# ruc-aimc-lab/GeoFormer

Measured on AMD Instinct MI355X. Metric: image-pairs/sec (640x640), higher is better.
Workload: dtype f16

## Files before the change

### geoformer_amd/_lib.py

```python
import ctypes
import os

_HERE = os.path.dirname(os.path.abspath(__file__))
LIB_PATH = os.environ.get('GF_LIB_PATH') or os.path.join(_HERE, 'libgeoformer_hip.so')

GF_F32, GF_F16, GF_BF16 = 0, 1, 2
GF_IMAGE_U8, GF_IMAGE_F32_NORMALISED, GF_IMAGE_F32_NORMALISED_RCP = 0, 1, 2

c_void_p, c_int, c_float, c_size_t = ctypes.c_void_p, ctypes.c_int, ctypes.c_float, ctypes.c_size_t
c_long, c_uint32 = ctypes.c_long, ctypes.c_uint32

SIGNATURES = {
    'gf_abi_version': (c_int, []),
    'gf_last_error': (ctypes.c_char_p, []),
    'gf_profile_filter': (None, [ctypes.c_char_p]),
    'gf_profile_enable': (None, [c_int]),
    'gf_profile_collect': (c_int, [ctypes.c_char_p, ctypes.POINTER(ctypes.c_double), ctypes.POINTER(c_int),
                                   ctypes.POINTER(ctypes.c_double)]),
    'gf_dual_softmax_workspace_bytes': (c_size_t, [c_int, c_int, c_int]),
    'gf_dual_softmax_match_only_supported': (c_int, [c_int, c_int, c_int, c_int, c_int, c_int]),
    'gf_dual_softmax_conf_at': (c_int, [c_void_p, c_void_p, c_int, c_int, c_int, c_int, c_int, c_float, c_void_p, c_void_p, c_void_p, c_int,
                                        c_void_p, c_void_p, c_size_t, c_void_p]),
    'gf_dual_softmax_match': (c_int, [c_void_p, c_void_p, c_int, c_int, c_int, c_int, c_int, c_void_p, c_void_p,
                                      c_float, c_float, c_int, c_int, c_int, c_float, c_void_p, c_void_p, c_void_p,
# ... 28 lines not shown
    'gf_coarse_loss_backward': (c_int, [c_int, c_int, c_int, c_int, c_void_p, c_void_p, c_float, c_void_p, c_void_p, c_void_p, c_int, c_void_p, c_float,
                                         c_void_p, c_void_p, c_void_p, c_void_p, c_size_t, c_void_p]),
    'gf_pos_encode': (c_int, [c_void_p, c_int, c_long, c_long, c_long, c_long, c_void_p, c_void_p, c_int, c_int, c_int,
                              c_int, c_int, c_void_p]),
    'gf_linear_attention_workspace_bytes': (c_size_t, [c_int, c_int, c_int, c_int]),
    'gf_linear_attention': (c_int, [c_void_p, c_void_p, c_void_p, c_int, c_int, c_int, c_int, c_int, c_int, c_long,
                                    c_long, c_long, c_void_p, c_void_p, c_float, c_void_p, c_void_p, c_size_t,
                                    c_void_p]),
    'gf_encoder_kv_workspace_bytes': (c_size_t, [c_int, c_int]),
    'gf_encoder_kv_state': (c_int, [c_void_p, c_long, c_int, c_int, c_int, c_void_p, c_void_p, c_void_p, c_void_p, c_size_t, c_void_p]),
    'gf_encoder_layer': (c_int, [c_void_p, c_long, c_void_p, c_long, c_void_p, c_int, c_void_p, c_float, c_void_p, c_void_p, c_float,
                                 c_float, c_int, c_void_p, c_int, c_void_p, c_long, c_int, c_int, c_int, c_void_p]),
    'gf_encoder_layer_kv': (c_int, [c_void_p, c_long, c_void_p, c_int, c_void_p, c_float, c_void_p, c_void_p, c_float, c_float, c_int,
                                    c_void_p, c_long, c_int, c_int, c_int, c_void_p, c_int, c_void_p, c_void_p, c_size_t, c_void_p]),
    'gf_fine_layer': (c_int, [c_void_p, c_void_p, c_void_p, c_int, c_int, c_int, c_void_p, c_void_p, c_float, c_float, c_float, c_void_p]),
    'gf_conv3x3_supported': (c_int, [c_int, c_int]),
    'gf_conv3x3s2_supported': (c_int, [c_int, c_int]),
    'gf_lateral_supported': (c_int, [c_int, c_int]),
    'gf_lateral_upsample_add_nhwc': (c_int, [c_void_p, c_void_p, c_void_p, c_void_p, c_int, c_int, c_int, c_int, c_int, c_int, c_int, c_int, c_void_p]),
    'gf_conv3x3_nhwc': (c_int, [c_void_p, c_void_p, c_void_p, c_void_p, c_void_p, c_void_p, c_int, c_int, c_int, c_int, c_int, c_int,
                                c_float, c_int, c_void_p]),
    'gf_linear': (c_int, [c_void_p, c_long, c_int, c_void_p, c_long, c_int, c_void_p, c_void_p, c_void_p, c_int, c_int,
                          c_void_p, c_void_p, c_float, c_void_p, c_long, c_void_p, c_int, c_void_p, c_long, c_int, c_int,
                          c_int, c_void_p]),
    'gf_ransac_workspace_bytes': (c_size_t, [c_int, c_int]),
    'gf_ransac_homography': (c_int, [c_void_p, c_void_p, c_void_p, c_int, c_int, c_float, c_void_p, c_void_p, c_float,
                                     c_int, c_uint32, c_int, c_int, c_void_p, c_void_p, c_void_p, c_void_p, c_void_p, c_void_p,
                                     c_void_p, c_void_p, c_size_t, c_void_p]),
    'gf_ransac_homography_v2': (c_int, [c_void_p, c_void_p, c_void_p, c_int, c_int, c_float, c_void_p, c_void_p, c_float,
                                        c_int, c_uint32, c_int, c_int, c_void_p, c_void_p, c_void_p, c_void_p, c_void_p, c_void_p,
# ... 115 lines not shown
```

### geoformer_amd/csrc/k11_fine_layer.hip

```cpp
#include <math.h>

#include <type_traits>

#include "gf_common.h"

#ifndef K11_TRACE
#define K11_TRACE 0
#endif
#if K11_TRACE
__device__ long long k11_trace[256 * 8 * 4 * 8];
#define K11_T(slot) do { if ((ln & 63) == 0 && blockIdx.x < 256 && git < 4) k11_trace[((blockIdx.x * 8 + wave) * 4 + git) * 8 + (slot)] = (long long)__builtin_amdgcn_s_memtime(); } while (0)
extern "C" int gf_debug_k11_trace(long long* out) {
    return (int)hipMemcpyFromSymbol(out, HIP_SYMBOL(k11_trace), sizeof(long long) * 256 * 8 * 4 * 8);
}
#else
#define K11_T(slot)
#endif

namespace {

constexpr int FC = 128;
#ifndef K11_FW
#define K11_FW 8
#endif
constexpr int FW = K11_FW;
static_assert(FW == 8 || FW == 4, "a weight block is 4 FW fragments: every wave moves four of them");
constexpr int FRAG = 1024, WBLK = 4 * FW * FRAG;
constexpr int NBLK = 320 / (4 * FW);
constexpr int TILE = 8192;
constexpr int X_OFF = 0;
constexpr int W_OFF = FW * TILE;
constexpr int VEC_OFF = W_OFF + 2 * WBLK;
constexpr int LDS_BYTES = VEC_OFF + 4 * FC * 4;

struct FlArgs {
    const void* x;
    const void* src;
    void* out;
    const void* wstream;
    const float* ln;
    float eps1, eps2, attn_eps;
    int Nw, Lw, groups;
};

template <typename T>
__device__ __forceinline__ typename Mma32<T>::Frag fl_pack8(float a0, float a1, float a2, float a3, float a4, float a5, float a6, float a7) {
    typename Mma32<T>::Frag f;
    f[0] = gf_from_float<T>(a0); f[1] = gf_from_float<T>(a1); f[2] = gf_from_float<T>(a2); f[3] = gf_from_float<T>(a3);
    f[4] = gf_from_float<T>(a4); f[5] = gf_from_float<T>(a5); f[6] = gf_from_float<T>(a6); f[7] = gf_from_float<T>(a7);
    return f;
}
template <typename T>
__device__ __forceinline__ typename Mma32<T>::Frag fl_pack_step(const v16f& a, int s) {
    return s == 0 ? fl_pack8<T>(a[0], a[1], a[2], a[3], a[4], a[5], a[6], a[7])
                  : fl_pack8<T>(a[8], a[9], a[10], a[11], a[12], a[13], a[14], a[15]);
}
__device__ __forceinline__ float fl_phi(float x) {
    return fmaxf(x, 0.f) + __builtin_amdgcn_fmed3f(__builtin_amdgcn_exp2f(x * 1.44269504088896341f), 0.f, 1.f);
}
template <typename T>
__device__ __forceinline__ float fl_rnd(float x) { return gf_to_float(gf_from_float<T>(x)); }

__device__ __forceinline__ v16f fl_zero() { return v16f{0.f, 0.f, 0.f, 0.f, 0.f, 0.f, 0.f, 0.f, 0.f, 0.f, 0.f, 0.f, 0.f, 0.f, 0.f, 0.f}; }

struct FlRing {
    GfRsrc ws;
    char* smem;
    int wave, lane;
    int blk;
    int sblk;
    int total;
};
__device__ __forceinline__ void fl_dma_block(const FlRing& r, int g, int sb) {
    char* dst = r.smem + W_OFF + (g & 1) * WBLK + r.wave * 4 * FRAG;
#pragma unroll
    for (int i = 0; i < 4; ++i) gf_lds_dma(r.ws, dst + i * FRAG, r.lane * 16, sb * WBLK + (r.wave * 4 + i) * FRAG);
    __builtin_amdgcn_sched_barrier(0);
}
template <typename Frag>
__device__ __forceinline__ void fl_load_step(const FlRing& r, Frag (&f)[4], int g, int st) {
    const char* p = r.smem + W_OFF + (g & 1) * WBLK + st * 4 * FRAG + r.lane * 16;
#pragma unroll
    for (int i = 0; i < 4; ++i) f[i] = *reinterpret_cast<const Frag*>(p + i * FRAG);
}
template <typename Frag>
__device__ __forceinline__ void fl_fetch_next(FlRing& r, Frag (&nx)[4], int st) {
    if (st == FW - 1) {
        asm volatile("s_waitcnt vmcnt(0) lgkmcnt(0)" ::: "memory");
        __builtin_amdgcn_s_barrier();
        if (r.blk + 2 < r.total) {
            int sb = r.sblk + 2;
            sb = sb >= NBLK ? sb - NBLK : sb;
            fl_dma_block(r, r.blk + 2, sb);
        }
        if (r.blk + 1 < r.total) fl_load_step(r, nx, r.blk + 1, 0);
        ++r.blk;
        r.sblk = r.sblk + 1 == NBLK ? 0 : r.sblk + 1;
    } else {
        fl_load_step(r, nx, r.blk, st + 1);
    }
}

__device__ __forceinline__ void fl_tile_dma(const GfRsrc& wins, int win_byte_offset, int Lw, char* tile, int lane) {
#pragma unroll
    for (int i = 0; i < 8; ++i) {
        const int row = 8 * (i & 3) + (lane >> 3), slot = lane & 7, c = slot ^ ((row >> 1) & 7);
        const int r = row < Lw ? row : Lw - 1;
        gf_lds_dma(wins, tile + i * FRAG, r * (FC * 2) + (i >> 2) * 128 + c * 16, win_byte_offset);
    }
}

template <typename T>
__global__ __launch_bounds__(64 * FW, 2) void fine_layer(FlArgs a) {
    using Mm = Mma32<T>;
    using Frag = typename Mm::Frag;
    extern __shared__ __attribute__((aligned(16))) char smem[];
    const int tid = threadIdx.x, lane = tid & 63, wave = __builtin_amdgcn_readfirstlane(tid >> 6);
    float* vec = reinterpret_cast<float*>(smem + VEC_OFF);
    char* tile = smem + X_OFF + wave * TILE;
#ifdef K11_PRIO
    if (wave >= 4) __builtin_amdgcn_s_setprio(1);
#endif
    const int my_groups = (a.groups - (int)blockIdx.x + (int)gridDim.x - 1) / (int)gridDim.x;
    FlRing ring{gf_rsrc(a.wstream, (unsigned)NBLK * WBLK), smem, wave, lane, 0, 0, my_groups * NBLK};
    const GfRsrc xrs = gf_rsrc(a.x, (unsigned)a.Nw * a.Lw * (FC * 2)), srs = gf_rsrc(a.src, (unsigned)a.Nw * a.Lw * (FC * 2));
    fl_dma_block(ring, 0, 0);
    fl_dma_block(ring, 1, 1);
    for (int i = tid; i < 4 * FC; i += 64 * FW) vec[i] = a.ln[i];
    const bool same_src = a.src == a.x;
    const float inv_s = 1.0f / (float)a.Lw, eps_s = a.attn_eps * inv_s;
    Frag ones;
#pragma unroll
    for (int j = 0; j < 8; ++j) ones[j] = gf_from_float<T>(1.0f);
    Frag fa[4], fb[4];
    bool first = true;

#define FL_STEP_BEGIN(gs)                                               \
    Frag (&cur)[4] = ((gs) & 1) ? fb : fa;                               \
    Frag (&nxt)[4] = ((gs) & 1) ? fa : fb;                               \
    fl_fetch_next(ring, nxt, (gs) & (FW - 1))

    int git = -1;
    (void)git;
    for (int g = blockIdx.x; g < a.groups; g += gridDim.x) {
        ++git;
        int ln = lane;
        asm volatile("" : "+v"(ln));
        const int h2 = ln >> 5, lr = ln & 31;
        v4u pm0, pm1;
#pragma unroll
        for (int p4 = 0; p4 < 4; ++p4) {
            const int ra = 8 * (p4 >> 1) + 4 * h2 + 2 * (p4 & 1);
            pm0[p4] = (ra < a.Lw ? 0xFFFFu : 0u) | (ra + 1 < a.Lw ? 0xFFFF0000u : 0u);
            pm1[p4] = (ra + 16 < a.Lw ? 0xFFFFu : 0u) | (ra + 17 < a.Lw ? 0xFFFF0000u : 0u);
        }
        auto tok_mask = [](const Frag& f, const v4u& m) { return __builtin_bit_cast(Frag, __builtin_bit_cast(v4u, f) & m); };
        const int win = g * FW + wave;
        K11_T(0);
        const int wclamp = win < a.Nw ? win : a.Nw - 1;
        const int win_off = (int)((unsigned)wclamp * (unsigned)(a.Lw * (FC * 2)));
        asm volatile("s_waitcnt lgkmcnt(0)" ::: "memory");
        fl_tile_dma(srs, win_off, a.Lw, tile, ln);
        if (first) {
            asm volatile("s_waitcnt vmcnt(0) lgkmcnt(0)" ::: "memory");
            __builtin_amdgcn_s_barrier();
            fl_load_step(ring, fa, 0, 0);
            first = false;
        } else {
            asm volatile("s_waitcnt vmcnt(0)" ::: "memory");
        }
        K11_T(1);
        Frag xf[8];
        auto load_xf = [&]() {
#pragma unroll
            for (int ks = 0; ks < 8; ++ks) {
                const int ch = 2 * ks + h2;
                xf[ks] = *reinterpret_cast<const Frag*>(tile + (ch >> 3) * 4096 + gf_lds_off(lr, ch & 7));
            }
        };
        load_xf();
        if (!same_src) {
            asm volatile("s_waitcnt lgkmcnt(0)" ::: "memory");
            fl_tile_dma(xrs, win_off, a.Lw, tile, ln);
        }

        Frag kvA[4][2], ksA[4][2];
#pragma unroll
        for (int nb = 0; nb < 4; ++nb) {
            v16f k = fl_zero(), v = fl_zero();
#pragma unroll
            for (int hf = 0; hf < 2; ++hf)
                {
                    FL_STEP_BEGIN(4 * nb + hf);
#pragma unroll
                    for (int i = 0; i < 4; ++i) Mm::mma(xf[4 * hf + i], cur[i], k);
// ... 97 lines not shown
                        for (int i = 0; i < 4; ++i) Mm::mma(cur[i], mB[2 * hf + (i >> 1)][i & 1], m[nb]);
                    }
            }
            float mean, rstd;
            ln_stats(m, a.eps1, mean, rstd);
#pragma unroll
            for (int nb = 0; nb < 4; ++nb)
#pragma unroll
                for (int sx = 0; sx < 2; ++sx) {
                    const v4f lo = ln_apply(m[nb], nb, 2 * sx, vec, vec + FC, mean, rstd), hi = ln_apply(m[nb], nb, 2 * sx + 1, vec, vec + FC, mean, rstd);
                    mB[nb][sx] = fl_pack8<T>(lo.x, lo.y, lo.z, lo.w, hi.x, hi.y, hi.z, hi.w);
                }
        }

        K11_T(4);
        v16f o[4];
#pragma unroll
        for (int nb = 0; nb < 4; ++nb) o[nb] = fl_zero();
#pragma unroll 1
        for (int hq = 0; hq < 2; ++hq) {
#pragma unroll
            for (int hb = 0; hb < 4; ++hb) {
                v16f hd = fl_zero();
#pragma unroll
                for (int hf = 0; hf < 2; ++hf)
                    {
                    FL_STEP_BEGIN(6 * hb + hf);
#pragma unroll
                        for (int i = 0; i < 4; ++i) Mm::mma(cur[i], xf[4 * hf + i], hd);
                    }
// ... 28 lines not shown
#pragma unroll
            for (int nb = 0; nb < 4; ++nb)
#pragma unroll
                for (int g4 = 0; g4 < 4; ++g4) {
                    const int c = nb * 32 + 8 * g4 + 4 * h2, ch = c >> 3;
                    char* p = tile + (ch >> 3) * 4096 + gf_lds_off(lr, ch & 7) + (c & 7) * 2;
                    const v4t xv = *reinterpret_cast<const v4t*>(p);
                    const v4f y = ln_apply(o[nb], nb, g4, vec + 2 * FC, vec + 3 * FC, mean2, rstd2);
                    v4t ov;
                    ov[0] = gf_from_float<T>(gf_to_float(xv[0]) + fl_rnd<T>(y.x));
                    ov[1] = gf_from_float<T>(gf_to_float(xv[1]) + fl_rnd<T>(y.y));
                    ov[2] = gf_from_float<T>(gf_to_float(xv[2]) + fl_rnd<T>(y.z));
                    ov[3] = gf_from_float<T>(gf_to_float(xv[3]) + fl_rnd<T>(y.w));
                    *reinterpret_cast<v4t*>(p) = ov;
                }
            __builtin_amdgcn_fence(__ATOMIC_RELEASE, "wavefront");
            __builtin_amdgcn_wave_barrier();
            __builtin_amdgcn_fence(__ATOMIC_ACQUIRE, "wavefront");
            if (win < a.Nw) {
                char* og = (char*)a.out + (size_t)win * a.Lw * (FC * 2);
#pragma unroll
                for (int i = 0; i < 8; ++i) {
                    const int e = ln + 64 * i, row = e >> 4, ch = e & 15;
                    if (row < a.Lw)
                        *reinterpret_cast<v4u*>(og + row * (FC * 2) + ch * 16) =
                            *reinterpret_cast<const v4u*>(tile + (ch >> 3) * 4096 + gf_lds_off(row, ch & 7));
                }
            }
        }
        K11_T(6);
    }
#undef FL_STEP_BEGIN
    asm volatile("s_waitcnt vmcnt(0) lgkmcnt(0)" ::: "memory");
}

}

extern "C" int gf_fine_layer(const void* x, const void* src, void* out, int dtype, int Nw, int Lw, const void* wstream,
                             const float* ln_params, float eps1, float eps2, float attn_eps, void* stream) {
    GF_CHECK_ARG(x && src && out && wstream && ln_params, "null pointer");
    GF_CHECK_ARG(Nw > 0, "empty problem");
    GF_CHECK_ARG(Lw > 0 && Lw <= 32, "windows of 1 .. 32 tokens");
    GF_CHECK_ARG(dtype == GF_F16 || dtype == GF_BF16, "the fused fine-level layer is built for 16-bit storage (GF_F16 / GF_BF16)");
    GF_CHECK_ARG((uintptr_t)x % 16 == 0 && (uintptr_t)src % 16 == 0 && (uintptr_t)out % 16 == 0 && (uintptr_t)wstream % 16 == 0,
                 "tensors must be 16-byte aligned");
    static std::atomic<uint64_t> attr{0};
    if (gf_first_use_on_device(attr)) {
        (void)hipFuncSetAttribute((const void*)fine_layer<_Float16>, hipFuncAttributeMaxDynamicSharedMemorySize, LDS_BYTES);
        (void)hipFuncSetAttribute((const void*)fine_layer<gf_bf16>, hipFuncAttributeMaxDynamicSharedMemorySize, LDS_BYTES);
    }
    hipStream_t st = (hipStream_t)stream;
    const double per_tok = 8.0 * FC * FC + 8.0 * FC * 16 + 8.0 * FC * FC + 4.0 * FC * FC;
    void* pt = gf_prof_begin("fine_layer", st, per_tok * (double)Nw * Lw);
    const long win_bytes = (long)Lw * FC * 2;
    const int per_launch = (int)(((1l << 31) - 65536) / win_bytes);
    for (long w0 = 0; w0 < Nw; w0 += per_launch) {
        const int nw = (int)((Nw - w0) < per_launch ? (Nw - w0) : per_launch);
        FlArgs a{(const char*)x + w0 * win_bytes, (const char*)src + w0 * win_bytes, (char*)out + w0 * win_bytes, wstream, ln_params,
                 eps1, eps2, attn_eps, nw, Lw, (nw + FW - 1) / FW};
        const int slots = 256 * (8 / FW), grid = a.groups < slots ? a.groups : slots;
        if (dtype == GF_F16) fine_layer<_Float16><<<grid, 64 * FW, LDS_BYTES, st>>>(a);
        else fine_layer<gf_bf16><<<grid, 64 * FW, LDS_BYTES, st>>>(a);
    }
    gf_prof_end("fine_layer", pt, st);
    GF_CHECK_LAUNCH();
    return GF_OK;
}
```

### geoformer_amd/fused.py

```python
import ctypes

import torch

from . import _lib
from ._lib import check
from .ops import _DTYPES, _contig, _dt, _need_cuda, _p, _rows2d, _stream, _ws

_IDX = {}


def _frag_index(order, device):
    key = (order, str(device))
    if key not in _IDX:
        lane = torch.arange(64, device=device)[:, None]
        j = torch.arange(8, device=device)[None, :]
        h = lane >> 5
        if order == 'std':
            koff = 8 * h + j
        else:
            koff = 8 * (j >> 2) + 4 * h + (j & 3)
        _IDX[key] = (koff, (lane & 31).expand(64, 8))
    return _IDX[key]


# ... 109 lines not shown
        for f in (fk, fv):
            parts += [_steps(f, one(nb), [h]) for h in halves]
    for f in (fq, fm):
        for nb in range(4):
            parts += [_steps(f, one(nb), [h]) for h in halves]
    f1x, f1m, f2 = fragments(w1[:, :c], 'std'), fragments(w1[:, c:], 'perm'), fragments(w2, 'perm')
    for hb in range(8):
        parts += [_steps(f1x, one(hb), [h]) for h in halves]
        parts += [_steps(f1m, one(hb), [h]) for h in halves]
        parts += [_steps(f2, all4, [[2 * hb + s]]) for s in range(2)]
    out = torch.cat(parts).contiguous()
    assert out.numel() == 10 * 32 * 64 * 8
    return out


def fine_layer(x, src, wstream, ln_params, eps1, eps2, attn_eps=1e-6, out=None):
    _need_cuda(x, src, wstream, ln_params)
    Nw, Lw, C = x.shape
    if C != 128 or src.shape != x.shape or x.dtype != src.dtype:
        raise ValueError('gf_fine_layer: x and src must be [Nw, Lw, 128] tensors of one 16-bit dtype')
    x = _contig(x)
    src = x if src is x else _contig(src)
    if out is None:
        out = torch.empty_like(x)
    elif out.shape != x.shape or out.dtype != x.dtype or not out.is_contiguous():
        raise ValueError('out must be a contiguous tensor of the result shape and dtype')
    if Nw == 0:
        return out
    check(_lib.lib().gf_fine_layer(_p(x), _p(src), _p(out), _dt(x), Nw, Lw, _p(wstream), _p(ln_params), float(eps1), float(eps2),
                                   float(attn_eps), _stream()), 'gf_fine_layer')
# ... 115 lines not shown
```

### geoformer_amd/model/full_model.py

```python
from typing import Dict, NamedTuple, Optional, Tuple

import torch
import torch.nn as nn

from .. import ops
from .backbone import build_backbone
from .geo_config import default_cfg
from .modules import (CoarseMatching, FineMatching2, FinePreprocess, GeoModule, LocalFeatureTransformer,
                      PositionEncodingSine, materialize_matches)

_PRECISIONS = {'fp32': (torch.float32, torch.float32), 'fp16': (torch.float16, torch.float16),
               'bf16': (torch.bfloat16, torch.bfloat16), 'bf16_fp16': (torch.float16, torch.bfloat16)}
PRECISIONS = tuple(_PRECISIONS)


_CONCURRENT_BACKBONES = [True]


class ImageFeatures(NamedTuple):
    coarse: torch.Tensor
    fine: torch.Tensor
    image_size: Tuple[int, int]

    @property
# ... 171 lines not shown

    def forward_static(self, data):
        img0, img1 = data['image0'], data['image1']
        data.update({'bs': torch.tensor(img0.size(0)), 'hw0_i': torch.tensor(img0.shape[2:]), 'hw1_i': torch.tensor(img1.shape[2:])})
        n = img0.size(0)
        if img0.shape[2:] == img1.shape[2:]:
            feats_c, feats_f = self._backbone(torch.cat([img0, img1], dim=0))
            (feat_c0, feat_c1), (feat_f0, feat_f1) = feats_c.split(n), feats_f.split(n)
        else:
            (feat_c0, feat_f0), (feat_c1, feat_f1) = self._backbone_unequal(img0, img1)
        return self.forward_features(data, feat_c0, feat_f0, feat_c1, feat_f1, static_only=True)

    def forward_dynamic(self, data):
        st = data.pop('_static')
        data.update(materialize_matches(st['raw']))
        f0u, f1u = self.fine_preprocess(st['feat_f0'], st['feat_f1'], st['geo0'], st['geo1'], data)
        if f0u.size(0) != 0:
            f0u, f1u = self.loftr_fine(f0u, f1u)
        self.fine_matching(f0u, f1u, data)
        data['_feat_dev'] = {'loftr_f0': st['feat0'], 'loftr_f1': st['feat1'], 'geo_f0': st['geo0'], 'geo_f1': st['geo1'],
                             'fine_f0': f0u, 'fine_f1': f1u}
        return data

    def forward_features(self, data, feat_c0, feat_f0, feat_c1, feat_f1, static_only=False):
        dt = self.compute_dtype
        data.update({'hw0_c': torch.tensor(feat_c0.shape[2:]), 'hw1_c': torch.tensor(feat_c1.shape[2:]),
                     'hw0_f': torch.tensor(feat_f0.shape[2:]), 'hw1_f': torch.tensor(feat_f1.shape[2:])})
        if 'bs' not in data:
            data.update({'bs': torch.tensor(data['image0'].size(0)), 'hw0_i': torch.tensor(data['image0'].shape[2:]),
                         'hw1_i': torch.tensor(data['image1'].shape[2:])})
        pe_both = None
        mo0, mo1 = data.pop('_pe_mask_out', (None, None))
        if feat_c0.shape == feat_c1.shape:
# ... 37 lines not shown
```

### geoformer_amd/model/modules.py

```python
import copy
import math
from typing import Dict, Optional

import torch
import torch.nn as nn
from .. import fused, ops


class PositionEncodingSine(nn.Module):

    def __init__(self, d_model, max_shape=(256, 256), temp_bug_fix=False):
        super().__init__()
        self.d_model, self.max_shape, self.temp_bug_fix = d_model, tuple(max_shape), temp_bug_fix
        self._tables = {}

    def table(self, h, w, device):
        key = (h, w, str(device))
        if key not in self._tables:
            if h > self.max_shape[0] or w > self.max_shape[1]:
                raise ValueError(f'feature map {h}x{w} exceeds max_shape {self.max_shape}')
            c = self.d_model
            ypos = torch.ones(h, w).cumsum(0).float().unsqueeze(0)
            xpos = torch.ones(h, w).cumsum(1).float().unsqueeze(0)
            k2 = torch.arange(0, c // 2, 2).float()
# ... 102 lines not shown
        if (x_mask is None and source_mask is None and x.shape == source.shape and self.fusable_window(x.dtype, x.shape[1])
                and x.is_contiguous() and source.is_contiguous()):
            w = self.weights(x.dtype)
            return fused.fine_layer(x, source, w['stream_fine'], w['ln'], self.norm1.eps, self.norm2.eps, out=out)
        if self.fusable(x.dtype):
            w = self.weights(x.dtype)
            state = fused.encoder_kv_state(source, w['stream_kv'], source_mask)
            return fused.encoder_layer(x, w['stream'], w['ln'], self.norm1.eps, self.norm2.eps,
                                       0 if self.activation == 'relu' else 1, kv_state=state, source_len=source.shape[1],
                                       q_mask=x_mask, out=out)
        q = self.project_q(x)
        k, v = self.project_kv(source)
        message = ops.linear_attention(q, k, v, self.nhead, x_mask, source_mask)
        return self.finish(x, message, out=out)

    def kv_state(self, source, source_mask=None, out=None):
        return fused.encoder_kv_state(source, self.weights(source.dtype)['stream_kv'], source_mask, out=out)

    def forward_state(self, x, state, source_len, x_mask=None, out=None, tail_layer=None, tail_first=0, tail_out=None):
        w = self.weights(x.dtype)
        tail = None if tail_layer is None else tail_layer.weights(x.dtype)['stream_kv']
        return fused.encoder_layer(x, w['stream'], w['ln'], self.norm1.eps, self.norm2.eps, 0 if self.activation == 'relu' else 1,
                                   kv_state=state, source_len=source_len, q_mask=x_mask, out=out, tail_stream=tail,
                                   tail_first=tail_first, tail_out=tail_out)


def _adjacent_halves(a, b):
    if (a.shape != b.shape or a.dtype != b.dtype or not a.is_contiguous() or not b.is_contiguous() or a.numel() == 0
            or a.untyped_storage().data_ptr() != b.untyped_storage().data_ptr()
            or b.storage_offset() != a.storage_offset() + a.numel()):
# ... 3 lines not shown

class LocalFeatureTransformer(nn.Module):

    def __init__(self, config):
        super().__init__()
        self.config = config
        self.d_model, self.nhead, self.layer_names = config['d_model'], config['nhead'], config['layer_names']
        if config['attention'] != 'linear':
            raise NotImplementedError("only attention='linear' (the GeoFormer configuration) is built")
        layer = LoFTREncoderLayer(config['d_model'], config['nhead'], 'linear', 'relu')
        self.layers = nn.ModuleList([copy.deepcopy(layer) for _ in self.layer_names])
        for p in self.parameters():
            if p.dim() > 1:
                nn.init.xavier_uniform_(p)

    def forward(self, feat0, feat1, mask0: Optional[torch.Tensor] = None, mask1: Optional[torch.Tensor] = None,
                both: Optional[torch.Tensor] = None):
        assert self.d_model == feat0.size(2), 'the feature number of src and transformer must be equal'
        same = feat0.shape == feat1.shape
        n = feat0.shape[0]
        if not same:
            both = None
        elif both is None:
            both = _adjacent_halves(feat0, feat1)
            if both is None:
                both = torch.cat([feat0, feat1], 0)
        mboth = torch.cat([mask0, mask1], 0) if (same and mask0 is not None) else None
        if same and both.is_cuda and all(ly.fusable(both.dtype) for ly in self.layers):
            return self._forward_fused(both, n, mask0, mask1, mboth)
        if (not same and feat0.is_cuda and feat0.dim() == 3 and feat0.shape[0] == feat1.shape[0]
                and all(ly.fusable(feat0.dtype) for ly in self.layers)):
            return self._forward_fused_unequal(feat0, feat1, mask0, mask1)
        for layer, name in zip(self.layers, self.layer_names):
            if name == 'self':
                if same:
                    both = layer(both, both, mboth, mboth)
                else:
                    feat0 = layer(feat0, feat0, mask0, mask0)
                    feat1 = layer(feat1, feat1, mask1, mask1)
            elif name == 'cross':
                if same:
                    nxt = torch.empty_like(both)
                    layer(both[:n], both[n:], mask0, mask1, out=nxt[:n])
                    layer(both[n:], nxt[:n], mask1, mask0, out=nxt[n:])
                    both = nxt
                else:
                    feat0 = layer(feat0, feat1, mask0, mask1)
                    feat1 = layer(feat1, feat0, mask1, mask0)
# ... 251 lines not shown
            geo['nidx_both'] = geo['nidx_t'].view(-1)
        geo['ransac'] = rs
        return geo

    def forward(self, cnn_desc0, cnn_desc1, batch, desc_map0=None, desc_map1=None, dtype=None, desc_both=None):
        n = cnn_desc0.shape[0]
        hw0c, hw1c = tuple(cnn_desc0.shape[2:]), tuple(cnn_desc1.shape[2:])
        if desc_map0 is None:
            desc_map0 = self.pos_encoding(cnn_desc0, dtype)
            desc_map1 = self.pos_encoding(cnn_desc1, dtype)
        geo = self.geometry(batch, n, hw0c, hw1c, cnn_desc0.device)
        batch['_geo_dev'] = geo
        return self.des_transformer(desc_map0, desc_map1, geo, both=desc_both)


class FinePreprocess(nn.Module):
    def __init__(self, config):
        super().__init__()
        self.config = config
        self.cat_c_feat = config['fine_concat_coarse_feat']
        self.W = config['fine_window_size']
        d_c, d_f = config['coarse']['d_model'], config['fine']['d_model']
        self.d_model_f = d_f
        if not self.cat_c_feat:
            raise NotImplementedError('GeoFormer always concatenates the coarse context (cvpr_ds_config.py:13)')
        self.down_proj = nn.Linear(d_c, d_f, bias=True)
        self.merge_feat = nn.Linear(2 * d_f, d_f, bias=True)
        for p in self.parameters():
            if p.dim() > 1:
                nn.init.kaiming_normal_(p, mode='fan_out', nonlinearity='relu')
# ... 2 lines not shown
    def invalidate(self):
        self._cache = {}

    def weights(self, dtype):
        w = self._cache.get(dtype)
        if w is None:
            d = self.d_model_f
            mw = self.merge_feat.weight.detach()
            w = {'dw': self.down_proj.weight.detach().to(dtype).contiguous(),
                 'db': self.down_proj.bias.detach().float().contiguous(),
                 'mw_win': mw[:, :d].to(dtype).contiguous(), 'mw_ctx': mw[:, d:].to(dtype).contiguous(),
                 'mb': self.merge_feat.bias.detach().float().contiguous()}
            self._cache[dtype] = w
        return w

    def forward(self, feat_f0, feat_f1, feat_c0, feat_c1, data: Dict[str, torch.Tensor]):
        W = self.W
        stride = int(data['hw0_f'][0]) // int(data['hw0_c'][0])
        data.update({'W': torch.tensor(W)})
        dtype = feat_c0.dtype
        M = data['b_ids'].shape[0]
        if M == 0:
            e = torch.empty(0, W ** 2, self.d_model_f, device=feat_f0.device, dtype=dtype)
            return e, e.clone()
        w = self.weights(dtype)
        ids = (data['b_ids'], data['i_ids'], data['j_ids'], int(data['hw0_c'][1]), int(data['hw1_c'][1]), stride, W)
        rows16 = (feat_f0.shape[1] == w['mw_win'].shape[1] and feat_c0.shape[-1] == feat_c1.shape[-1] == w['dw'].shape[1]
                  and ops.fine_rows_supported(feat_f0, feat_f1, dtype))
        if rows16:
            fc0, fc1 = feat_c0.contiguous(), feat_c1.contiguous()
            rows16 = fc0.data_ptr() % 16 == 0 and fc1.data_ptr() % 16 == 0 and fc0.shape[-1] % 64 == 0
        if rows16:
            win_rows, c_rows = ops.fine_rows(feat_f0, feat_f1, fc0, fc1, *ids, supported=True)
            ctx = ops.linear(ops.linear_rows(c_rows, w['dw'], bias=w['db']), w['mw_ctx'], bias=w['mb'])
            out = ops.linear_rows(win_rows, w['mw_win'], rowgroup_bias=ctx, rowgroup_rows=W * W)
            return out[:M], out[M:]
        win, ccat = ops.fine_gather(feat_f0, feat_f1, feat_c0, feat_c1, *ids, dtype)
        ctx = ops.linear(ops.linear(ccat, w['dw'], bias=w['db']), w['mw_ctx'], bias=w['mb'])
        out = ops.linear(win, w['mw_win'], rowgroup_bias=ctx, rowgroup_rows=W * W)
        return out[:M], out[M:]


class FineMatching2(nn.Module):
    def __init__(self, temperature=0.1, thr=0.1):
        super().__init__()
        self.temperature, self.thr = temperature, thr

    def forward(self, feat_f0, feat_f1, data: Dict[str, torch.Tensor]):
        M, WW, C = feat_f0.shape
# ... 11 lines not shown
```

### include/geoformer_hip.h

```cpp
#ifndef GEOFORMER_HIP_H_
#define GEOFORMER_HIP_H_

#include <stddef.h>
#include <stdint.h>

#ifdef __cplusplus
extern "C" {
#endif

typedef enum { GF_OK = 0, GF_ERR_INVALID_ARGUMENT = -1, GF_ERR_WORKSPACE = -2, GF_ERR_LAUNCH = -3 } gf_status;
typedef enum { GF_F32 = 0, GF_F16 = 1, GF_BF16 = 2 } gf_dtype;

#define GF_ABI_VERSION 4
int gf_abi_version(void);
const char* gf_last_error(void);

void gf_profile_enable(int on);
void gf_profile_filter(const char* tag);
int gf_profile_collect(const char* tag, double* total_ms, int* count, double* work);

size_t gf_dual_softmax_workspace_bytes(int N, int L, int S);
int gf_dual_softmax_match_only_supported(int dtype, int L, int S, int C, int masked, int force_one);
int gf_dual_softmax_conf_at(const void* f0, const void* f1, int dtype, int N, int L, int S, int C, float temperature,
                            const int64_t* b, const int64_t* i, const int64_t* j, int P, float* out, void* workspace,
// ... 57 lines not shown
size_t gf_encoder_kv_workspace_bytes(int N, int S);
int gf_encoder_kv_state(const void* src, long ld, int dtype, int N, int S, const uint8_t* kv_mask,
                        const void* wstream_kv, float* kv_state, void* workspace, size_t workspace_bytes,
                        void* stream);
int gf_encoder_layer(const void* x, long ldx, const void* msg, long ldm, const float* kv_state, int S,
                     const uint8_t* q_mask, float attn_eps, const void* wstream, const float* ln_params, float eps1,
                     float eps2, int activation, const int32_t* row_flag, int flag_rows, void* out, long ldo, int dtype,
                     int N, int L, void* stream);
int gf_encoder_layer_kv(const void* x, long ldx, const float* kv_state, int S, const uint8_t* q_mask, float attn_eps,
                        const void* wstream, const float* ln_params, float eps1, float eps2, int activation, void* out,
                        long ldo, int dtype, int N, int L, const void* wstream_tail, int tail_first, float* kv_state_out,
                        void* workspace, size_t workspace_bytes, void* stream);

int gf_fine_layer(const void* x, const void* src, void* out, int dtype, int Nw, int Lw, const void* wstream,
                  const float* ln_params, float eps1, float eps2, float attn_eps, void* stream);

#define GF_CONV_PAD16 0x100
#define GF_CONV_REM8 0x200
#define GF_CONV_S2 0x400
int gf_conv3x3_supported(int cin, int cout);
int gf_conv3x3s2_supported(int cin, int cout);
int gf_conv3x3_nhwc(const void* x, const void* wstream, const float* shift, const void* residual, void* out,
                    const void* zeros, int N, int H, int W, int cin, int cout, int act, float slope, int dtype,
                    void* stream);

int gf_linear(const void* a1, long lda1, int k1, const void* a2, long lda2, int k2, const void* w,
              const float* bias, const void* rowgroup_bias, int rowgroup_rows, int epilogue,
              const float* ln_gamma, const float* ln_beta, float ln_eps, const void* residual, long ldres,
              const int32_t* row_flag, int flag_rows, void* out, long ldo, int dtype, int M, int N,
              void* stream);
// ... 168 lines not shown
```

Baseline: 758.2.

## Fuse fine-window projection GEMM into the first fine transformer layer kernel

Adds a ROWS variant of the fused fine-layer kernel that gathers window rows by address, runs the window projection GEMM plus per-window context bias in-kernel, and writes the result into the LDS tile before the attention layer. The projection weights are prepended to the layer's weight stream. This removes the separate linear_rows launch and the round trip of its output through global memory. The cost is extra in-kernel GEMM work, a prefetch of the next window's rows, and higher register pressure.

```diff
diff --git a/geoformer_amd/_lib.py b/geoformer_amd/_lib.py
--- a/geoformer_amd/_lib.py
+++ b/geoformer_amd/_lib.py
@@ -66,6 +66,7 @@
     'gf_encoder_layer_kv': (c_int, [c_void_p, c_long, c_void_p, c_int, c_void_p, c_float, c_void_p, c_void_p, c_float, c_float, c_int,
                                     c_void_p, c_long, c_int, c_int, c_int, c_void_p, c_int, c_void_p, c_void_p, c_size_t, c_void_p]),
     'gf_fine_layer': (c_int, [c_void_p, c_void_p, c_void_p, c_int, c_int, c_int, c_void_p, c_void_p, c_float, c_float, c_float, c_void_p]),
+    'gf_fine_layer_rows': (c_int, [c_void_p, c_void_p, c_void_p, c_int, c_int, c_int, c_void_p, c_void_p, c_float, c_float, c_float, c_void_p]),
     'gf_conv3x3_supported': (c_int, [c_int, c_int]),
     'gf_conv3x3s2_supported': (c_int, [c_int, c_int]),
     'gf_lateral_supported': (c_int, [c_int, c_int]),
diff --git a/geoformer_amd/csrc/k11_fine_layer.hip b/geoformer_amd/csrc/k11_fine_layer.hip
--- a/geoformer_amd/csrc/k11_fine_layer.hip
+++ b/geoformer_amd/csrc/k11_fine_layer.hip
@@ -27,6 +27,7 @@
 static_assert(FW == 8 || FW == 4, "a weight block is 4 FW fragments: every wave moves four of them");
 constexpr int FRAG = 1024, WBLK = 4 * FW * FRAG;
 constexpr int NBLK = 320 / (4 * FW);
+constexpr int PBLK = 32 / (4 * FW);
 constexpr int TILE = 8192;
 constexpr int X_OFF = 0;
 constexpr int W_OFF = FW * TILE;
@@ -41,6 +42,8 @@
     const float* ln;
     float eps1, eps2, attn_eps;
     int Nw, Lw, groups;
+    const unsigned long long* rows;
+    const void* ctx;
 };
 
 template <typename T>
@@ -70,6 +73,7 @@
     int blk;
     int sblk;
     int total;
+    int nblk;
 };
 __device__ __forceinline__ void fl_dma_block(const FlRing& r, int g, int sb) {
     char* dst = r.smem + W_OFF + (g & 1) * WBLK + r.wave * 4 * FRAG;
@@ -90,12 +94,12 @@
         __builtin_amdgcn_s_barrier();
         if (r.blk + 2 < r.total) {
             int sb = r.sblk + 2;
-            sb = sb >= NBLK ? sb - NBLK : sb;
+            sb = sb >= r.nblk ? sb - r.nblk : sb;
             fl_dma_block(r, r.blk + 2, sb);
         }
         if (r.blk + 1 < r.total) fl_load_step(r, nx, r.blk + 1, 0);
         ++r.blk;
-        r.sblk = r.sblk + 1 == NBLK ? 0 : r.sblk + 1;
+        r.sblk = r.sblk + 1 == r.nblk ? 0 : r.sblk + 1;
     } else {
         fl_load_step(r, nx, r.blk, st + 1);
     }
@@ -110,7 +114,45 @@
     }
 }
 
-template <typename T>
+typedef const __attribute__((address_space(1))) char* FlGlobal;
+struct FlRowsReq {
+    unsigned long long addr[4];
+    v4u piece[8];
+    gf_v2u ctx[16];
+    unsigned live;
+};
+__device__ __forceinline__ void fl_rows_addresses(FlRowsReq& rq, const unsigned long long* rows, int Lw, int lane) {
+#pragma unroll
+    for (int q = 0; q < 4; ++q) {
+        const int row = 8 * q + (lane >> 3);
+        rq.addr[q] = rows[row < Lw ? row : Lw - 1];
+    }
+}
+__device__ __forceinline__ void fl_rows_request(FlRowsReq& rq, const void* ctx_row, int lane) {
+    const FlGlobal cx = (FlGlobal)(unsigned long long)ctx_row;
+    FlGlobal src[4];
+    rq.live = 0;
+#pragma unroll
+    for (int q = 0; q < 4; ++q) {
+        rq.live |= rq.addr[q] ? 1u << q : 0u;
+        src[q] = rq.addr[q] ? (FlGlobal)rq.addr[q] : cx;
+    }
+#pragma unroll
+    for (int i = 0; i < 8; ++i) {
+        const int row = 8 * (i & 3) + (lane >> 3), slot = lane & 7, c = slot ^ ((row >> 1) & 7);
+        rq.piece[i] = *reinterpret_cast<const __attribute__((address_space(1))) v4u*>(src[i & 3] + (i >> 2) * 128 + c * 16);
+    }
+#pragma unroll
+    for (int e = 0; e < 16; ++e)
+        rq.ctx[e] = *reinterpret_cast<const __attribute__((address_space(1))) gf_v2u*>(cx + ((e >> 2) * 32 + 8 * (e & 3) + 4 * (lane >> 5)) * 2);
+}
+__device__ __forceinline__ void fl_rows_stage(const FlRowsReq& rq, char* tile, int lane) {
+#pragma unroll
+    for (int i = 0; i < 8; ++i)
+        *reinterpret_cast<v4u*>(tile + i * FRAG + lane * 16) = (rq.live >> (i & 3) & 1) ? rq.piece[i] : v4u{0u, 0u, 0u, 0u};
+}
+
+template <typename T, bool ROWS>
 __global__ __launch_bounds__(64 * FW, 2) void fine_layer(FlArgs a) {
     using Mm = Mma32<T>;
     using Frag = typename Mm::Frag;
@@ -122,18 +164,32 @@
     if (wave >= 4) __builtin_amdgcn_s_setprio(1);
 #endif
     const int my_groups = (a.groups - (int)blockIdx.x + (int)gridDim.x - 1) / (int)gridDim.x;
-    FlRing ring{gf_rsrc(a.wstream, (unsigned)NBLK * WBLK), smem, wave, lane, 0, 0, my_groups * NBLK};
+    constexpr int SBLK = NBLK + (ROWS ? PBLK : 0);
+    FlRing ring{gf_rsrc(a.wstream, (unsigned)SBLK * WBLK), smem, wave, lane, 0, 0, my_groups * SBLK, SBLK};
     const GfRsrc xrs = gf_rsrc(a.x, (unsigned)a.Nw * a.Lw * (FC * 2)), srs = gf_rsrc(a.src, (unsigned)a.Nw * a.Lw * (FC * 2));
     fl_dma_block(ring, 0, 0);
     fl_dma_block(ring, 1, 1);
     for (int i = tid; i < 4 * FC; i += 64 * FW) vec[i] = a.ln[i];
-    const bool same_src = a.src == a.x;
+    const bool same_src = ROWS || a.src == a.x;
     const float inv_s = 1.0f / (float)a.Lw, eps_s = a.attn_eps * inv_s;
     Frag ones;
 #pragma unroll
     for (int j = 0; j < 8; ++j) ones[j] = gf_from_float<T>(1.0f);
     Frag fa[4], fb[4];
     bool first = true;
+    FlRowsReq rq;
+    auto rows_addresses = [&](int w, int ln) {
+        w = w < a.Nw ? w : a.Nw - 1;
+        fl_rows_addresses(rq, a.rows + (size_t)w * a.Lw, a.Lw, ln);
+    };
+    auto rows_request = [&](int w, int ln) {
+        w = w < a.Nw ? w : a.Nw - 1;
+        fl_rows_request(rq, reinterpret_cast<const char*>(a.ctx) + (size_t)w * (FC * 2), ln);
+    };
+    if constexpr (ROWS) {
+        rows_addresses((int)blockIdx.x * FW + wave, lane);
+        rows_request((int)blockIdx.x * FW + wave, lane);
+    }
 
 #define FL_STEP_BEGIN(gs)                                               \
     Frag (&cur)[4] = ((gs) & 1) ? fb : fa;                               \
@@ -145,6 +201,11 @@
     for (int g = blockIdx.x; g < a.groups; g += gridDim.x) {
         ++git;
         int ln = lane;
+        if constexpr (ROWS) {
+            int z = 0;
+            asm volatile("" : "+v"(z));
+            ln = __builtin_amdgcn_mbcnt_hi(~0u, __builtin_amdgcn_mbcnt_lo(~0u, z));
+        }
         asm volatile("" : "+v"(ln));
         const int h2 = ln >> 5, lr = ln & 31;
         v4u pm0, pm1;
@@ -160,15 +221,22 @@
         const int wclamp = win < a.Nw ? win : a.Nw - 1;
         const int win_off = (int)((unsigned)wclamp * (unsigned)(a.Lw * (FC * 2)));
         asm volatile("s_waitcnt lgkmcnt(0)" ::: "memory");
-        fl_tile_dma(srs, win_off, a.Lw, tile, ln);
+        if constexpr (ROWS) fl_rows_stage(rq, tile, ln);
+        else fl_tile_dma(srs, win_off, a.Lw, tile, ln);
         if (first) {
             asm volatile("s_waitcnt vmcnt(0) lgkmcnt(0)" ::: "memory");
             __builtin_amdgcn_s_barrier();
             fl_load_step(ring, fa, 0, 0);
             first = false;
-        } else {
+        } else if constexpr (!ROWS) {
             asm volatile("s_waitcnt vmcnt(0)" ::: "memory");
         }
+        auto tile_written = []() {
+            __builtin_amdgcn_fence(__ATOMIC_RELEASE, "wavefront");
+            __builtin_amdgcn_wave_barrier();
+            __builtin_amdgcn_fence(__ATOMIC_ACQUIRE, "wavefront");
+        };
+        if constexpr (ROWS) tile_written();
         K11_T(1);
         Frag xf[8];
         auto load_xf = [&]() {
@@ -179,6 +247,32 @@
             }
         };
         load_xf();
+        if constexpr (ROWS) {
+            typedef T v4t __attribute__((ext_vector_type(4)));
+#pragma unroll
+            for (int nb = 0; nb < 4; ++nb) {
+                v16f w = fl_zero();
+#pragma unroll
+                for (int hf = 0; hf < 2; ++hf)
+                    {
+                    FL_STEP_BEGIN(2 * nb + hf);
+#pragma unroll
+                        for (int i = 0; i < 4; ++i) Mm::mma(cur[i], xf[4 * hf + i], w);
+                    }
+#pragma unroll
+                for (int g4 = 0; g4 < 4; ++g4) {
+                    const int c = nb * 32 + 8 * g4 + 4 * h2, ch = c >> 3;
+                    const v4t cb = __builtin_bit_cast(v4t, rq.ctx[4 * nb + g4]);
+                    v4t ov;
+#pragma unroll
+                    for (int j = 0; j < 4; ++j) ov[j] = gf_from_float<T>(w[4 * g4 + j] + 0.f + gf_to_float(cb[j]));
+                    *reinterpret_cast<v4t*>(tile + (ch >> 3) * 4096 + gf_lds_off(lr, ch & 7) + (c & 7) * 2) = ov;
+                }
+            }
+            tile_written();
+            load_xf();
+            K11_T(7);
+        }
         if (!same_src) {
             asm volatile("s_waitcnt lgkmcnt(0)" ::: "memory");
             fl_tile_dma(xrs, win_off, a.Lw, tile, ln);
@@ -306,6 +400,7 @@
         }
 
         K11_T(4);
+        if constexpr (ROWS) rows_addresses((g + (int)gridDim.x) * FW + wave, ln);
         v16f o[4];
 #pragma unroll
         for (int nb = 0; nb < 4; ++nb) o[nb] = fl_zero();
@@ -364,9 +459,8 @@
                     ov[3] = gf_from_float<T>(gf_to_float(xv[3]) + fl_rnd<T>(y.w));
                     *reinterpret_cast<v4t*>(p) = ov;
                 }
-            __builtin_amdgcn_fence(__ATOMIC_RELEASE, "wavefront");
-            __builtin_amdgcn_wave_barrier();
-            __builtin_amdgcn_fence(__ATOMIC_ACQUIRE, "wavefront");
+            tile_written();
+            if constexpr (ROWS) rows_request((g + (int)gridDim.x) * FW + wave, ln);
             if (win < a.Nw) {
                 char* og = (char*)a.out + (size_t)win * a.Lw * (FC * 2);
 #pragma unroll
@@ -383,6 +477,22 @@
 #undef FL_STEP_BEGIN
     asm volatile("s_waitcnt vmcnt(0) lgkmcnt(0)" ::: "memory");
 }
+
+}
+
+namespace {
+
+void fl_set_attributes() {
+    static std::atomic<uint64_t> attr{0};
+    if (gf_first_use_on_device(attr)) {
+        (void)hipFuncSetAttribute((const void*)fine_layer<_Float16, false>, hipFuncAttributeMaxDynamicSharedMemorySize, LDS_BYTES);
+        (void)hipFuncSetAttribute((const void*)fine_layer<gf_bf16, false>, hipFuncAttributeMaxDynamicSharedMemorySize, LDS_BYTES);
+        (void)hipFuncSetAttribute((const void*)fine_layer<_Float16, true>, hipFuncAttributeMaxDynamicSharedMemorySize, LDS_BYTES);
+        (void)hipFuncSetAttribute((const void*)fine_layer<gf_bf16, true>, hipFuncAttributeMaxDynamicSharedMemorySize, LDS_BYTES);
+    }
+}
+constexpr double FL_FLOPS_PER_TOKEN = 8.0 * FC * FC + 8.0 * FC * 16 + 8.0 * FC * FC + 4.0 * FC * FC;
+constexpr int fl_grid(int groups) { return groups < 256 * (8 / FW) ? groups : 256 * (8 / FW); }
 
 }
 
@@ -394,25 +504,40 @@
     GF_CHECK_ARG(dtype == GF_F16 || dtype == GF_BF16, "the fused fine-level layer is built for 16-bit storage (GF_F16 / GF_BF16)");
     GF_CHECK_ARG((uintptr_t)x % 16 == 0 && (uintptr_t)src % 16 == 0 && (uintptr_t)out % 16 == 0 && (uintptr_t)wstream % 16 == 0,
                  "tensors must be 16-byte aligned");
-    static std::atomic<uint64_t> attr{0};
-    if (gf_first_use_on_device(attr)) {
-        (void)hipFuncSetAttribute((const void*)fine_layer<_Float16>, hipFuncAttributeMaxDynamicSharedMemorySize, LDS_BYTES);
-        (void)hipFuncSetAttribute((const void*)fine_layer<gf_bf16>, hipFuncAttributeMaxDynamicSharedMemorySize, LDS_BYTES);
-    }
+    fl_set_attributes();
     hipStream_t st = (hipStream_t)stream;
-    const double per_tok = 8.0 * FC * FC + 8.0 * FC * 16 + 8.0 * FC * FC + 4.0 * FC * FC;
-    void* pt = gf_prof_begin("fine_layer", st, per_tok * (double)Nw * Lw);
+    void* pt = gf_prof_begin("fine_layer", st, FL_FLOPS_PER_TOKEN * (double)Nw * Lw);
     const long win_bytes = (long)Lw * FC * 2;
     const int per_launch = (int)(((1l << 31) - 65536) / win_bytes);
     for (long w0 = 0; w0 < Nw; w0 += per_launch) {
         const int nw = (int)((Nw - w0) < per_launch ? (Nw - w0) : per_launch);
         FlArgs a{(const char*)x + w0 * win_bytes, (const char*)src + w0 * win_bytes, (char*)out + w0 * win_bytes, wstream, ln_params,
-                 eps1, eps2, attn_eps, nw, Lw, (nw + FW - 1) / FW};
-        const int slots = 256 * (8 / FW), grid = a.groups < slots ? a.groups : slots;
-        if (dtype == GF_F16) fine_layer<_Float16><<<grid, 64 * FW, LDS_BYTES, st>>>(a);
-        else fine_layer<gf_bf16><<<grid, 64 * FW, LDS_BYTES, st>>>(a);
+                 eps1, eps2, attn_eps, nw, Lw, (nw + FW - 1) / FW, nullptr, nullptr};
+        const int grid = fl_grid(a.groups);
+        if (dtype == GF_F16) fine_layer<_Float16, false><<<grid, 64 * FW, LDS_BYTES, st>>>(a);
+        else fine_layer<gf_bf16, false><<<grid, 64 * FW, LDS_BYTES, st>>>(a);
     }
     gf_prof_end("fine_layer", pt, st);
     GF_CHECK_LAUNCH();
     return GF_OK;
 }
+
+extern "C" int gf_fine_layer_rows(const uint64_t* win_rows, const void* ctx, void* out, int dtype, int Nw, int Lw, const void* wstream,
+                                  const float* ln_params, float eps1, float eps2, float attn_eps, void* stream) {
+    GF_CHECK_ARG(win_rows && ctx && out && wstream && ln_params, "null pointer");
+    GF_CHECK_ARG(Nw > 0, "empty problem");
+    GF_CHECK_ARG(Lw > 0 && Lw <= 32, "windows of 1 .. 32 tokens");
+    GF_CHECK_ARG(dtype == GF_F16 || dtype == GF_BF16, "the fused fine-level layer is built for 16-bit storage (GF_F16 / GF_BF16)");
+    GF_CHECK_ARG((uintptr_t)win_rows % 8 == 0, "the row table must be 8-byte aligned");
+    GF_CHECK_ARG((uintptr_t)ctx % 16 == 0 && (uintptr_t)out % 16 == 0 && (uintptr_t)wstream % 16 == 0, "tensors must be 16-byte aligned");
+    fl_set_attributes();
+    hipStream_t st = (hipStream_t)stream;
+    void* pt = gf_prof_begin("fine_layer", st, (FL_FLOPS_PER_TOKEN + 2.0 * FC * FC) * (double)Nw * Lw);
+    FlArgs a{nullptr, nullptr, out, wstream, ln_params, eps1, eps2, attn_eps, Nw, Lw, (Nw + FW - 1) / FW,
+             (const unsigned long long*)win_rows, ctx};
+    if (dtype == GF_F16) fine_layer<_Float16, true><<<fl_grid(a.groups), 64 * FW, LDS_BYTES, st>>>(a);
+    else fine_layer<gf_bf16, true><<<fl_grid(a.groups), 64 * FW, LDS_BYTES, st>>>(a);
+    gf_prof_end("fine_layer", pt, st);
+    GF_CHECK_LAUNCH();
+    return GF_OK;
+}
diff --git a/geoformer_amd/fused.py b/geoformer_amd/fused.py
--- a/geoformer_amd/fused.py
+++ b/geoformer_amd/fused.py
@@ -147,6 +147,33 @@
     return out
 
 
+def pack_fine_rows_stream(w_win, layer_stream):
+    if w_win.shape != (128, 128) or w_win.dtype != layer_stream.dtype:
+        raise ValueError('the fused window GEMM is built for a [128, 128] weight of the layer\'s 16-bit dtype')
+    f = fragments(w_win, 'std')
+    parts = [_steps(f, torch.tensor([nb], device=w_win.device), [h]) for nb in range(4) for h in ([0, 1, 2, 3], [4, 5, 6, 7])]
+    return torch.cat(parts + [layer_stream]).contiguous()
+
+
+def fine_layer_rows(win_rows, ctx, wstream, ln_params, eps1, eps2, attn_eps=1e-6, out=None):
+    _need_cuda(win_rows, ctx, wstream, ln_params)
+    if win_rows.dim() != 2 or win_rows.dtype != torch.int64 or not win_rows.is_contiguous():
+        raise ValueError('gf_fine_layer_rows: win_rows must be a contiguous int64 [Nw, Lw] tensor of addresses')
+    Nw, Lw = win_rows.shape
+    if ctx.shape != (Nw, 128) or ctx.dtype not in (torch.float16, torch.bfloat16) or wstream.dtype != ctx.dtype:
+        raise ValueError('gf_fine_layer_rows: ctx must be [Nw, 128] of the 16-bit dtype of the stream')
+    ctx = _contig(ctx)
+    if out is None:
+        out = torch.empty(Nw, Lw, 128, dtype=ctx.dtype, device=ctx.device)
+    elif out.shape != (Nw, Lw, 128) or out.dtype != ctx.dtype or not out.is_contiguous():
+        raise ValueError('out must be a contiguous tensor of the result shape and dtype')
+    if Nw == 0:
+        return out
+    check(_lib.lib().gf_fine_layer_rows(_p(win_rows), _p(ctx), _p(out), _dt(ctx), Nw, Lw, _p(wstream), _p(ln_params), float(eps1),
+                                        float(eps2), float(attn_eps), _stream()), 'gf_fine_layer_rows')
+    return out
+
+
 def fine_layer(x, src, wstream, ln_params, eps1, eps2, attn_eps=1e-6, out=None):
     _need_cuda(x, src, wstream, ln_params)
     Nw, Lw, C = x.shape
diff --git a/geoformer_amd/model/full_model.py b/geoformer_amd/model/full_model.py
--- a/geoformer_amd/model/full_model.py
+++ b/geoformer_amd/model/full_model.py
@@ -6,7 +6,7 @@
 from .. import ops
 from .backbone import build_backbone
 from .geo_config import default_cfg
-from .modules import (CoarseMatching, FineMatching2, FinePreprocess, GeoModule, LocalFeatureTransformer,
+from .modules import (CoarseMatching, FineMatching2, FinePreprocess, FineRows, GeoModule, LocalFeatureTransformer,
                       PositionEncodingSine, materialize_matches)
 
 _PRECISIONS = {'fp32': (torch.float32, torch.float32), 'fp16': (torch.float16, torch.float16),
@@ -209,9 +209,14 @@
     def forward_dynamic(self, data):
         st = data.pop('_static')
         data.update(materialize_matches(st['raw']))
-        f0u, f1u = self.fine_preprocess(st['feat_f0'], st['feat_f1'], st['geo0'], st['geo1'], data)
-        if f0u.size(0) != 0:
-            f0u, f1u = self.loftr_fine(f0u, f1u)
+        pre = self.fine_preprocess(st['feat_f0'], st['feat_f1'], st['geo0'], st['geo1'], data,
+                                   as_rows=self.loftr_fine.takes_rows(st['geo0'].dtype, self.fine_preprocess.W ** 2))
+        if isinstance(pre, FineRows):
+            f0u, f1u = self.loftr_fine.forward_rows(pre)
+        else:
+            f0u, f1u = pre
+            if f0u.size(0) != 0:
+                f0u, f1u = self.loftr_fine(f0u, f1u)
         self.fine_matching(f0u, f1u, data)
         data['_feat_dev'] = {'loftr_f0': st['feat0'], 'loftr_f1': st['feat1'], 'geo_f0': st['geo0'], 'geo_f1': st['geo1'],
                              'fine_f0': f0u, 'fine_f1': f1u}
diff --git a/geoformer_amd/model/modules.py b/geoformer_amd/model/modules.py
--- a/geoformer_amd/model/modules.py
+++ b/geoformer_amd/model/modules.py
@@ -1,6 +1,6 @@
 import copy
 import math
-from typing import Dict, Optional
+from typing import Dict, NamedTuple, Optional
 
 import torch
 import torch.nn as nn
@@ -140,6 +140,13 @@
         message = ops.linear_attention(q, k, v, self.nhead, x_mask, source_mask)
         return self.finish(x, message, out=out)
 
+    def forward_rows(self, fr, out=None):
+        w = self.weights(fr.ctx.dtype)
+        packed = w.get('stream_fine_rows')
+        if packed is None or packed[0] is not fr.w_win:
+            packed = w['stream_fine_rows'] = (fr.w_win, fused.pack_fine_rows_stream(fr.w_win, w['stream_fine']))
+        return fused.fine_layer_rows(fr.win_rows, fr.ctx, packed[1], w['ln'], self.norm1.eps, self.norm2.eps, out=out)
+
     def kv_state(self, source, source_mask=None, out=None):
         return fused.encoder_kv_state(source, self.weights(source.dtype)['stream_kv'], source_mask, out=out)
 
@@ -173,8 +180,16 @@
             if p.dim() > 1:
                 nn.init.xavier_uniform_(p)
 
+    def takes_rows(self, dtype, seq_len):
+        return bool(self.layer_names) and self.layer_names[0] == 'self' and self.layers[0].fusable_window(dtype, seq_len)
+
+    def forward_rows(self, fr):
+        both = self.layers[0].forward_rows(fr)
+        n = both.shape[0] // 2
+        return self.forward(both[:n], both[n:], both=both, first_layer=1)
+
     def forward(self, feat0, feat1, mask0: Optional[torch.Tensor] = None, mask1: Optional[torch.Tensor] = None,
-                both: Optional[torch.Tensor] = None):
+                both: Optional[torch.Tensor] = None, first_layer: int = 0):
         assert self.d_model == feat0.size(2), 'the feature number of src and transformer must be equal'
         same = feat0.shape == feat1.shape
         n = feat0.shape[0]
@@ -185,12 +200,12 @@
             if both is None:
                 both = torch.cat([feat0, feat1], 0)
         mboth = torch.cat([mask0, mask1], 0) if (same and mask0 is not None) else None
-        if same and both.is_cuda and all(ly.fusable(both.dtype) for ly in self.layers):
+        if first_layer == 0 and same and both.is_cuda and all(ly.fusable(both.dtype) for ly in self.layers):
             return self._forward_fused(both, n, mask0, mask1, mboth)
-        if (not same and feat0.is_cuda and feat0.dim() == 3 and feat0.shape[0] == feat1.shape[0]
+        if (first_layer == 0 and not same and feat0.is_cuda and feat0.dim() == 3 and feat0.shape[0] == feat1.shape[0]
                 and all(ly.fusable(feat0.dtype) for ly in self.layers)):
             return self._forward_fused_unequal(feat0, feat1, mask0, mask1)
-        for layer, name in zip(self.layers, self.layer_names):
+        for layer, name in list(zip(self.layers, self.layer_names))[first_layer:]:
             if name == 'self':
                 if same:
                     both = layer(both, both, mboth, mboth)
@@ -472,6 +487,13 @@
         return self.des_transformer(desc_map0, desc_map1, geo, both=desc_both)
 
 
+class FineRows(NamedTuple):
+    win_rows: torch.Tensor
+    ctx: torch.Tensor
+    w_win: torch.Tensor
+    maps: tuple
+
+
 class FinePreprocess(nn.Module):
     def __init__(self, config):
         super().__init__()
@@ -504,7 +526,7 @@
             self._cache[dtype] = w
         return w
 
-    def forward(self, feat_f0, feat_f1, feat_c0, feat_c1, data: Dict[str, torch.Tensor]):
+    def forward(self, feat_f0, feat_f1, feat_c0, feat_c1, data: Dict[str, torch.Tensor], as_rows: bool = False):
         W = self.W
         stride = int(data['hw0_f'][0]) // int(data['hw0_c'][0])
         data.update({'W': torch.tensor(W)})
@@ -523,6 +545,8 @@
         if rows16:
             win_rows, c_rows = ops.fine_rows(feat_f0, feat_f1, fc0, fc1, *ids, supported=True)
             ctx = ops.linear(ops.linear_rows(c_rows, w['dw'], bias=w['db']), w['mw_ctx'], bias=w['mb'])
+            if as_rows:
+                return FineRows(win_rows, ctx, w['mw_win'], (feat_f0, feat_f1))
             out = ops.linear_rows(win_rows, w['mw_win'], rowgroup_bias=ctx, rowgroup_rows=W * W)
             return out[:M], out[M:]
         win, ccat = ops.fine_gather(feat_f0, feat_f1, feat_c0, feat_c1, *ids, dtype)
diff --git a/include/geoformer_hip.h b/include/geoformer_hip.h
--- a/include/geoformer_hip.h
+++ b/include/geoformer_hip.h
@@ -95,6 +95,8 @@
 
 int gf_fine_layer(const void* x, const void* src, void* out, int dtype, int Nw, int Lw, const void* wstream,
                   const float* ln_params, float eps1, float eps2, float attn_eps, void* stream);
+int gf_fine_layer_rows(const uint64_t* win_rows, const void* ctx, void* out, int dtype, int Nw, int Lw, const void* wstream,
+                       const float* ln_params, float eps1, float eps2, float attn_eps, void* stream);
 
 #define GF_CONV_PAD16 0x100
 #define GF_CONV_REM8 0x200
```

Result: no change. 761.8, median of 6 (+0.5%).
